# youmi-zym/GO-SLAM

Hardware: NVIDIA H100
Metric: keyframe-BA-updates/s (higher is better)
Workload: dtype f16 corr (f32 accumulate) / f32 BA (f64 solve)

## Files before the change

go-slam_b200/csrc/corr_build_tc.cu:

```cuda
#include "common.cuh"
#include "tc_ptx.cuh"
#include <mutex>
#include <cstdio>
#include <cuda.h>
#include <cstdlib>
#include <cstring>

int gs_corr_build_simt_f16(const __half* f1, const __half* f2, __half* const* levels,
                           int num_levels, int N, int D, int h, int w, cudaStream_t st);

namespace {

constexpr int kD = 128;
constexpr int kBM = 128;
constexpr int kPY = 8, kPX = 16;
constexpr int kKBox = 64;
constexpr int kTileBytes = kBM * kD * 2;
constexpr int kBoxBytes = kBM * kKBox * 2;
constexpr int kBStages = 2;
constexpr int kGroupWarps = 4;
constexpr int kEpiThreads = 2 * kGroupWarps * 32;
constexpr int kThreadsTC = kEpiThreads + 128;
constexpr int kProducerRegs = 40, kConsumerRegs = 232;
constexpr int kMaxXB = 8;
constexpr int kBarBytes = 1024;
constexpr int kL0HalfBytes = 64 * 2 * 128;
constexpr int kL1HalfBytes = 64 * 64;
constexpr int kXpRowWords = 68;
constexpr int kXpWarpBytes = 8 * kXpRowWords * 4;
constexpr int kFixedBytes = 1024 + kBarBytes + (1 + kBStages) * kTileBytes;
__host__ __device__ constexpr int pitch2_of(int n_xb) { return (n_xb * 16 + 31) / 32 * 32; }
__host__ __device__ constexpr int pool2_src_bytes(bool tiled, int n_xb) {
  return tiled ? pitch2_of(n_xb) + 48 : 2 * n_xb * 8 + 8;
}
__host__ __device__ constexpr int pool1_src_bytes(int n_xb) { return 4 * n_xb * 16 + 16; }
__host__ __device__ constexpr int smem_bytes(bool tiled, int n_xb) {
  return tiled ? kFixedBytes + 2 * kBStages * (kL0HalfBytes + kL1HalfBytes) + kBM * pool2_src_bytes(true, n_xb)
               : kFixedBytes + kBM * (pool1_src_bytes(n_xb) + pool2_src_bytes(false, n_xb)) +
                     kEpiThreads / 32 * kXpWarpBytes;
}
static_assert(smem_bytes(true, kMaxXB) <= 227 * 1024 && smem_bytes(false, kMaxXB) <= 227 * 1024,
              "corr_build_tc_kernel exceeds the 227 KB of shared memory of a block");

using namespace gs_tc;

struct TcParams {
  __half* lvl[4];
  int num_levels, N, h, w, hw;
  int n_mt, n_yb, n_xb;
  int n_items;
  const int64_t* ii; const int64_t* jj; int rig;
  const int* out_slot;
  int w4_0, h4_0, w4_1, h4_1;
  int pitch2, pitch3;
  int aligned;
  int experiment;
};

__device__ __forceinline__ uint32_t pack2(float a, float b) {
  const __half2 h = __floats2half2_rn(a, b);
  return *reinterpret_cast<const uint32_t*>(&h);
}
__device__ __forceinline__ float lo_f(uint32_t u) {
  return __half2float(__ushort_as_half((unsigned short)(u & 0xffffu)));
}
__device__ __forceinline__ float hi_f(uint32_t u) {
  return __half2float(__ushort_as_half((unsigned short)(u >> 16)));
}
__device__ __forceinline__ float pool_pair(uint32_t top, uint32_t bot) {
  float s = lo_f(top);
  s += hi_f(top);
  s += lo_f(bot);
  s += hi_f(bot);
  return s * 0.25f;
}
template <int NW>
__device__ __forceinline__ void store_row(__half* dst, const uint32_t (&r)[NW], int nvalid) {
  const uintptr_t a = reinterpret_cast<uintptr_t>(dst);
  if (nvalid >= 2 * NW) {
    if (NW == 8 && (a & 31) == 0) {
      asm volatile("st.global.v4.b32 [%0], {%1,%2,%3,%4}; st.global.v4.b32 [%0+16], {%5,%6,%7,%8};" ::"l"(dst), "r"(r[0]),
                   "r"(r[1]), "r"(r[2]), "r"(r[3]), "r"(r[4]), "r"(r[5]), "r"(r[6]), "r"(r[7])
                   : "memory");
      return;
    }
    if (NW >= 4 && (a & 15) == 0) {
#pragma unroll
      for (int i = 0; i < NW; i += 4)
        *reinterpret_cast<uint4*>(dst + 2 * i) = make_uint4(r[i], r[i + 1], r[i + 2], r[i + 3]);
      return;
    }
    if (NW == 2 && (a & 7) == 0) {
      *reinterpret_cast<uint2*>(dst) = make_uint2(r[0], r[1]);
      return;
    }
    if ((a & 3) == 0) {
#pragma unroll
      for (int i = 0; i < NW; ++i) *reinterpret_cast<uint32_t*>(dst + 2 * i) = r[i];
      return;
    }
  }
#pragma unroll
  for (int i = 0; i < NW; ++i) {
    if (2 * i < nvalid) dst[2 * i] = __ushort_as_half((unsigned short)(r[i] & 0xffffu));
    if (2 * i + 1 < nvalid) dst[2 * i + 1] = __ushort_as_half((unsigned short)(r[i] >> 16));
  }
}

__device__ __forceinline__ void tiled_half_epilogue(const float (&acc)[2][32], unsigned char* st0, unsigned char* st1,
                                                    unsigned char* pool2_row0, int p2src, int p2row, int xb,
                                                    int wrow, int lane) {
  uint32_t W[2][2][4][2];
#pragma unroll
  for (int rh = 0; rh < 2; ++rh)
#pragma unroll
    for (int ty = 0; ty < 2; ++ty)
#pragma unroll
      for (int r4 = 0; r4 < 4; ++r4)
#pragma unroll
        for (int jx = 0; jx < 2; ++jx) {
          const int j = 2 * r4 + jx;
          W[rh][ty][r4][jx] = pack2(acc[ty][4 * j + 2 * rh], acc[ty][4 * j + 2 * rh + 1]);
        }
  {
    const bool lo = (lane & 3) < 2;
    const bool dflip = (lane >> 4) & 1;
    const int s8 = lane & 7;
    const uint32_t st0_u = smem_u32(st0);
#pragma unroll
    for (int a = 0; a < 2; ++a)
#pragma unroll
      for (int k = 0; k < 2; ++k)
#pragma unroll
        for (int jx = 0; jx < 2; ++jx) {
          uint32_t m[4];
#pragma unroll
          for (int rh = 0; rh < 2; ++rh) {
            const uint32_t ra = dflip ? W[rh][a ^ 1][2 * k][jx] : W[rh][a][2 * k][jx];
            const uint32_t rb = dflip ? W[rh][a ^ 1][2 * k + 1][jx] : W[rh][a][2 * k + 1][jx];
            const uint32_t recv = __shfl_xor_sync(0xffffffffu, lo ? rb : ra, 2);
            m[2 * rh] = lo ? ra : recv;
            m[2 * rh + 1] = lo ? recv : rb;
          }
          const int tya = a ^ (s8 >> 2);
          const int R = 2 * (wrow + 8 * (lane >> 4) + s8) + tya;
          const int chunk = 2 * (2 * jx + ((lane >> 3) & 1)) + k;
          stmatrix_x4(st0_u + R * 128 + ((chunk ^ (R & 7)) << 4), m);
        }
  }
  const bool ev = (lane & 1) == 0;
  const uint32_t st1_u = smem_u32(st1);
#pragma unroll
  for (int rh = 0; rh < 2; ++rh) {
    const int s = wrow + 8 * rh + (lane >> 2);
#pragma unroll
    for (int jx = 0; jx < 2; ++jx) {
      float v[4];
#pragma unroll
      for (int ty = 0; ty < 2; ++ty)
#pragma unroll
        for (int k = 0; k < 2; ++k) v[2 * ty + k] = pool_pair(W[rh][ty][2 * k][jx], W[rh][ty][2 * k + 1][jx]);
      const uint32_t own01 = pack2(v[0], v[1]), own23 = pack2(v[2], v[3]);
      const uint32_t recv = __shfl_xor_sync(0xffffffffu, ev ? own23 : own01, 1);
      const uint32_t mine = ev ? own01 : own23;
      const uint32_t lo_w = ev ? mine : recv, hi_w = ev ? recv : mine;
      const uint32_t w0 = __byte_perm(lo_w, hi_w, 0x5410);
      const uint32_t w1 = __byte_perm(lo_w, hi_w, 0x7632);
      const int chunk = (2 * jx + (lane & 1)) ^ ((s >> 1) & 3);
      const uint32_t a1 = st1_u + s * 64 + (chunk << 4) + ((lane & 3) >> 1) * 4;
      st_shared_u32(a1 + (ev ? 0 : 8), ev ? w0 : w1);
      st_shared_u32(a1 + (ev ? 8 : 0), ev ? w1 : w0);
      const uint32_t l2 = pack2(pool_pair(w0, w1), 0.f);
      st_shared_u16(smem_u32(pool2_row0 + s * p2src + (lane & 1) * p2row + xb * 8 + (2 * jx + ((lane & 3) >> 1)) * 2),
                    (uint16_t)(l2 & 0xffffu));
    }
  }
}

template <bool kTiled>
__global__ void __launch_bounds__(kThreadsTC, 1)
corr_build_tc_kernel(const __grid_constant__ CUtensorMap mapA, const __grid_constant__ CUtensorMap mapB,
                     const __grid_constant__ CUtensorMap mapL0, const __grid_constant__ CUtensorMap mapL1,
                     const TcParams p) {
  extern __shared__ unsigned char smem_raw[];
  unsigned char* base = smem_raw + ((1024u - (smem_u32(smem_raw) & 1023u)) & 1023u);
  uint64_t* bars = reinterpret_cast<uint64_t*>(base);
  unsigned char* smA = base + kBarBytes;
  unsigned char* smB = smA + kTileBytes;
  unsigned char* smEpi = smB + kBStages * kTileBytes;
  uint64_t* full_a = bars;
  uint64_t* empty_a = bars + 1;
  uint64_t* full_b = bars + 2;
  uint64_t* empty_b = full_b + kBStages;

  const int warp = threadIdx.x >> 5, lane = threadIdx.x & 31;

  if (threadIdx.x == 0) {
    mbar_init(full_a, 1); mbar_init(empty_a, kEpiThreads / 32);
    for (int i = 0; i < kBStages; ++i) { mbar_init(&full_b[i], 1); mbar_init(&empty_b[i], kGroupWarps); }
    fence_barrier_init();
  }
  __syncthreads();

  if (warp >= kEpiThreads / 32) {
    setmaxnreg_dec<kProducerRegs>();
    if (warp == kEpiThreads / 32 && lane == 0) {
      int aph = 0, bs = 0, bph = 0;
      for (int item = blockIdx.x; item < p.n_items; item += gridDim.x) {
        const int yb = item % p.n_yb;
        const int mt = (item / p.n_yb) % p.n_mt;
        const int n = item / (p.n_yb * p.n_mt);
        int n1 = n, n2 = n;
        if (p.ii != nullptr) {
          const int fi = (int)p.ii[n], fj = (int)p.jj[n];
          n1 = p.rig * fi;
          n2 = p.rig * fj + ((fi == fj && p.rig > 1) ? 1 : 0);
        }
        mbar_wait(empty_a, aph ^ 1);
        mbar_expect_tx(full_a, kTileBytes);
        tma_load_3d(&mapA, full_a, smA, 0, mt * kBM, n1);
        tma_load_3d(&mapA, full_a, smA + kBoxBytes, kKBox, mt * kBM, n1);
        aph ^= 1;
        for (int xb = 0; xb < p.n_xb; ++xb) {
          mbar_wait(&empty_b[bs], bph ^ 1);
          mbar_expect_tx(&full_b[bs], kTileBytes);
          tma_load_4d(&mapB, &full_b[bs], smB + bs * kTileBytes, 0, xb * kPX, yb * kPY, n2);
          tma_load_4d(&mapB, &full_b[bs], smB + bs * kTileBytes + kBoxBytes, kKBox, xb * kPX,
                      yb * kPY, n2);
          if (++bs == kBStages) { bs = 0; bph ^= 1; }
        }
      }
    }
  } else {
    setmaxnreg_inc<kConsumerRegs>();
    const int group = warp >> 2;
    const int half = lane >> 4;
    const int etid = threadIdx.x;
    const int ts = group;
    unsigned char* smL0 = smEpi;
    unsigned char* smL1 = smL0 + 2 * kBStages * kL0HalfBytes;
    const int p1row = p.n_xb * 16, p1src = pool1_src_bytes(p.n_xb);
    const int p2row = p.n_xb * 8;
    const int p2src = pool2_src_bytes(kTiled, p.n_xb);
    unsigned char* pool1 = smEpi;
    unsigned char* pool2 = kTiled ? smL1 + 2 * kBStages * kL1HalfBytes : pool1 + kBM * p1src;
    unsigned char* smXp = pool2 + kBM * p2src;
    uint32_t* xp = reinterpret_cast<uint32_t*>(smXp + warp * kXpWarpBytes);
    const int h1 = p.h >> 1, w1 = p.w >> 1, h2 = p.h >> 2, w2 = p.w >> 2, h3 = p.h >> 3, w3 = p.w >> 3;
    const bool wr = p.experiment != 1;
    const bool tma_thread = (etid & 127) == 0;
    if (kTiled && etid < kBM) {
      for (int b = 2 * p2row; b < p.pitch2; b += 4)
        *reinterpret_cast<uint32_t*>(pool2 + etid * p2src + b) = 0u;
    }
    int aph = 0, bph = 0, tile = 0;
    for (int item = blockIdx.x; item < p.n_items; item += gridDim.x) {
      const int yb = item % p.n_yb;
      const int mt = (item / p.n_yb) % p.n_mt;
      const int n = item / (p.n_yb * p.n_mt);
      const int n_out = p.out_slot ? __ldg(p.out_slot + n) : n;
      const int y0 = yb * kPY;
      mbar_wait(full_a, aph);
      aph ^= 1;
      bool a_held = true;
      for (int xb = 0; xb < p.n_xb; ++xb, ++tile) {
        if ((tile & (kBStages - 1)) != ts) continue;
        const int x0 = xb * kPX;
        mbar_wait(&full_b[ts], bph);
        bph ^= 1;
        float acc[2][2][32];
        {
          const uint32_t a_addr = smem_u32(smA);
          const uint32_t b_addr = smem_u32(smB + ts * kTileBytes);
          wgmma_fence();
#pragma unroll
          for (int kb = 0; kb < kD / kKBox; ++kb) {
#pragma unroll
            for (int k = 0; k < kKBox / 16; ++k) {
              const uint64_t db = make_desc_sw128(b_addr + kb * kBoxBytes + k * 32);
              const uint32_t on = (kb | k) != 0 ? 1u : 0u;
#pragma unroll
              for (int mh = 0; mh < 2; ++mh) {
                const uint64_t da = make_desc_sw128(a_addr + mh * 64 * 128 + kb * kBoxBytes + k * 32);
                wgmma_m64n64(acc[mh][0], da, db, on);
                wgmma_m64n64(acc[mh][1], da, db + ((64 * 128) >> 4), on);
              }
            }
          }
          wgmma_commit();
          wgmma_wait<0>();
        }
        __syncwarp();
        if (lane == 0) {
          mbar_arrive(&empty_b[ts]);
          if (xb + kBStages >= p.n_xb) mbar_arrive(empty_a);
        }
        if (xb + kBStages >= p.n_xb) a_held = false;
#pragma unroll
        for (int mh = 0; mh < 2; ++mh) {
        if constexpr (kTiled) {
          unsigned char* st0 = smL0 + (group * 2 + mh) * kL0HalfBytes;
          unsigned char* st1 = smL1 + (group * 2 + mh) * kL1HalfBytes;
          tiled_half_epilogue(acc[mh], st0, st1, pool2 + mh * 64 * p2src, p2src, p2row, xb, (warp & 3) * 16, lane);
          fence_async_smem();
          if (tma_thread) bulk_wait_read<0>();
          named_bar_sync(1 + group, 128);
          if (tma_thread) {
            const int s0 = mt * kBM + mh * 64;
            if (wr && s0 < p.hw) {
              tma_store_4d(&mapL0, st0, xb * 64, 2 * yb, s0, n_out);
              if (p.num_levels > 1 && yb < p.h4_1) tma_store_4d(&mapL1, st1, xb * 32, yb, s0, n_out);
            }
            bulk_commit();
          }
        } else {
        const int row = mh * 64 + (warp & 3) * 16 + (lane & 15);
        const int src = mt * kBM + row;
        const bool src_ok = src < p.hw && wr;
        const long long plane_id = (long long)n_out * p.hw + src;
        uint32_t hr[4][8];
#pragma unroll
        for (int pass = 0; pass < 2; ++pass) {
#pragma unroll
          for (int sub = 0; sub < 2; ++sub)
#pragma unroll
            for (int j = 0; j < 8; ++j)
              xp[(lane >> 2) * kXpRowWords + sub * 32 + 4 * j + (lane & 3)] =
                  pack2(acc[mh][sub][4 * j + 2 * pass], acc[mh][sub][4 * j + 2 * pass + 1]);
          __syncwarp();
          if (((lane >> 3) & 1) == pass) {
            const uint4* sp = reinterpret_cast<const uint4*>(xp + (lane & 7) * kXpRowWords + half * 32);
#pragma unroll
            for (int i = 0; i < 8; ++i) {
              const uint4 v = sp[i];
              hr[i >> 1][4 * (i & 1)] = v.x; hr[i >> 1][4 * (i & 1) + 1] = v.y;
              hr[i >> 1][4 * (i & 1) + 2] = v.z; hr[i >> 1][4 * (i & 1) + 3] = v.w;
            }
          }
          __syncwarp();
        }
        uint32_t l1[2][4];
#pragma unroll
        for (int cc = 0; cc < 2; ++cc) {
          const int c = 2 * half + cc;
          if (src_ok) {
#pragma unroll
            for (int r = 0; r < 2; ++r) {
              const int y = y0 + 2 * c + r;
              if (y < p.h) store_row<8>(p.lvl[0] + (plane_id * p.h + y) * p.w + x0, hr[2 * cc + r], p.w - x0);
            }
          }
#pragma unroll
          for (int j = 0; j < 4; ++j)
            l1[cc][j] = pack2(pool_pair(hr[2 * cc][2 * j], hr[2 * cc + 1][2 * j]),
                              pool_pair(hr[2 * cc][2 * j + 1], hr[2 * cc + 1][2 * j + 1]));
          *reinterpret_cast<uint4*>(pool1 + row * p1src + c * p1row + xb * 16) =
              make_uint4(l1[cc][0], l1[cc][1], l1[cc][2], l1[cc][3]);
        }
        {
          const uint32_t a0 = pack2(pool_pair(l1[0][0], l1[1][0]), pool_pair(l1[0][1], l1[1][1]));
          const uint32_t a1 = pack2(pool_pair(l1[0][2], l1[1][2]), pool_pair(l1[0][3], l1[1][3]));
          *reinterpret_cast<uint2*>(pool2 + row * p2src + half * p2row + xb * 8) = make_uint2(a0, a1);
        }
        }
        }
      }
      if (a_held && lane == 0) mbar_arrive(empty_a);
      if (kTiled) fence_async_smem();
      named_bar_sync(3, kEpiThreads);
      if (wr && p.num_levels > 1)
      for (int s_loc = etid >> 2; s_loc < kBM; s_loc += kEpiThreads / 4) {
        const int part = etid & 3;
        const int s_glb = mt * kBM + s_loc;
        if (s_glb < p.hw) {
          const long long pl = (long long)n_out * p.hw + s_glb;
          const unsigned char* sp1 = pool1 + s_loc * p1src;
          const unsigned char* sp2 = pool2 + s_loc * p2src;
          if constexpr (kTiled) {
            if (part == 1 && p.num_levels > 2 && 2 * yb < h2) {
              bulk_store(reinterpret_cast<unsigned char*>(p.lvl[2]) + (pl * p.n_yb + yb) * (long long)p.pitch2, sp2,
                         (uint32_t)p.pitch2);
              bulk_commit();
              bulk_wait_read();
            }
            if (part == 2 && p.num_levels > 3 && yb < h3) {
              unsigned char* s3 = const_cast<unsigned char*>(sp2) + p.pitch2;
#pragma unroll
              for (int k = 0; k < 8; ++k) {
                uint32_t v = 0u;
                if (k < p.n_xb) {
                  const uint32_t t = *reinterpret_cast<const uint32_t*>(sp2 + 8 * k);
                  const uint32_t t2 = *reinterpret_cast<const uint32_t*>(sp2 + 8 * k + 4);
                  const uint32_t b = *reinterpret_cast<const uint32_t*>(sp2 + p2row + 8 * k);
                  const uint32_t b2 = *reinterpret_cast<const uint32_t*>(sp2 + p2row + 8 * k + 4);
                  v = pack2(pool_pair(t, b), pool_pair(t2, b2));
                }
                reinterpret_cast<uint32_t*>(s3)[k] = v;
              }
              fence_async_smem();
              bulk_store(reinterpret_cast<unsigned char*>(p.lvl[3]) + (pl * p.n_yb + yb) * 32LL, s3, 32u);
              bulk_commit();
              bulk_wait_read();
            }
          } else if (p.aligned) {
            unsigned char* g1 = reinterpret_cast<unsigned char*>(p.lvl[1]) +
                                (pl * h1 + (y0 >> 1)) * (long long)p1row;
            for (int off = part * 32; off < 4 * p1row; off += 128) {
              uint32_t rr[8];
#pragma unroll
              for (int k = 0; k < 8; ++k) rr[k] = *reinterpret_cast<const uint32_t*>(sp1 + off + 4 * k);
              asm volatile("st.global.v4.b32 [%0], {%1,%2,%3,%4}; st.global.v4.b32 [%0+16], {%5,%6,%7,%8};" ::"l"(g1 + off), "r"(rr[0]),
                           "r"(rr[1]), "r"(rr[2]), "r"(rr[3]), "r"(rr[4]), "r"(rr[5]), "r"(rr[6]), "r"(rr[7])
                           : "memory");
            }
            if (part == 1 && p.num_levels > 2) {
              unsigned char* g2 = reinterpret_cast<unsigned char*>(p.lvl[2]) +
                                  (pl * h2 + (y0 >> 2)) * (long long)p2row;
              for (int off = 0; off < 2 * p2row; off += 16)
                *reinterpret_cast<uint4*>(g2 + off) = make_uint4(
                    *reinterpret_cast<const uint32_t*>(sp2 + off), *reinterpret_cast<const uint32_t*>(sp2 + off + 4),
                    *reinterpret_cast<const uint32_t*>(sp2 + off + 8), *reinterpret_cast<const uint32_t*>(sp2 + off + 12));
            }
            if (part == 2 && p.num_levels > 3) {
              __half* g3 = p.lvl[3] + (pl * h3 + (y0 >> 3)) * w3;
              for (int x = 0; x < w3; x += 2) {
                const uint32_t t = *reinterpret_cast<const uint32_t*>(sp2 + 4 * x);
                const uint32_t t2 = *reinterpret_cast<const uint32_t*>(sp2 + 4 * x + 4);
                const uint32_t b = *reinterpret_cast<const uint32_t*>(sp2 + p2row + 4 * x);
                const uint32_t b2 = *reinterpret_cast<const uint32_t*>(sp2 + p2row + 4 * x + 4);
                *reinterpret_cast<uint32_t*>(g3 + x) = pack2(pool_pair(t, b), pool_pair(t2, b2));
              }
            }
          } else {
            const __half* s1 = reinterpret_cast<const __half*>(sp1);
            const __half* s2 = reinterpret_cast<const __half*>(sp2);
            for (int r = 0; r < 4; ++r) {
              const int y = (y0 >> 1) + r;
              if (y >= h1) break;
              __half* g = p.lvl[1] + (pl * h1 + y) * w1;
              for (int x = part; x < w1; x += 4) g[x] = s1[r * (p1row / 2) + x];
            }
            if (p.num_levels > 2)
              for (int r = 0; r < 2; ++r) {
                const int y = (y0 >> 2) + r;
                if (y >= h2) break;
                __half* g = p.lvl[2] + (pl * h2 + y) * w2;
                for (int x = part; x < w2; x += 4) g[x] = s2[r * (p2row / 2) + x];
              }
            if (p.num_levels > 3 && (y0 >> 3) < h3) {
              __half* g = p.lvl[3] + (pl * h3 + (y0 >> 3)) * w3;
              for (int x = part; x < w3; x += 4) {
                float sum = __half2float(s2[2 * x]);
                sum += __half2float(s2[2 * x + 1]);
                sum += __half2float(s2[(p2row / 2) + 2 * x]);
                sum += __half2float(s2[(p2row / 2) + 2 * x + 1]);
                g[x] = __float2half_rn(sum * 0.25f);
              }
// ... 11 lines not shown
to_kmajor_kernel(const __half* __restrict__ in, __half* __restrict__ out, int hw) {
  __shared__ __align__(16) __half tile[kD][64 + 2];
  const int n = blockIdx.y;
  const int p0 = blockIdx.x * 64;
  const __half* src = in + (size_t)n * kD * hw;
  const __half q = __float2half_rn(0.25f);
  if ((hw & 7) == 0 && p0 + 64 <= hw) {
    const __half2 q2 = __half2half2(q);
    for (int idx = threadIdx.x; idx < kD * 8; idx += 256) {
      const int k = idx >> 3, pp = (idx & 7) * 8;
      uint4 v = __ldg(reinterpret_cast<const uint4*>(src + (size_t)k * hw + p0 + pp));
      __half2* h = reinterpret_cast<__half2*>(&v);
      uint32_t* dstw = reinterpret_cast<uint32_t*>(&tile[k][pp]);
#pragma unroll
      for (int u = 0; u < 4; ++u) {
        const __half2 r = __hmul2(h[u], q2);
        dstw[u] = *reinterpret_cast<const uint32_t*>(&r);
      }
    }
  } else {
    for (int idx = threadIdx.x; idx < kD * 64; idx += 256) {
      const int k = idx / 64, pp = idx % 64;
      tile[k][pp] = (p0 + pp < hw) ? __hmul(src[(size_t)k * hw + p0 + pp], q) : __half(0.f);
    }
  }
  __syncthreads();
  __half* dst = out + ((size_t)n * hw + p0) * kD;
  for (int idx = threadIdx.x; idx < 64 * (kD / 2); idx += 256) {
    const int pp = idx / (kD / 2), k2 = idx % (kD / 2);
    if (p0 + pp < hw) {
      __half2 v = __halves2half2(tile[2 * k2][pp], tile[2 * k2 + 1][pp]);
      reinterpret_cast<__half2*>(dst + (size_t)pp * kD)[k2] = v;
    }
  }
}

typedef CUresult (*EncodeTiledFn)(CUtensorMap*, CUtensorMapDataType, cuuint32_t, void*,
                                  const cuuint64_t*, const cuuint64_t*, const cuuint32_t*,
                                  const cuuint32_t*, CUtensorMapInterleave, CUtensorMapSwizzle,
                                  CUtensorMapL2promotion, CUtensorMapFloatOOBfill);

EncodeTiledFn get_encode_fn() {
  static EncodeTiledFn fn = nullptr;
  if (fn) return fn;
  void* p = nullptr;
  cudaDriverEntryPointQueryResult q;
  if (cudaGetDriverEntryPoint("cuTensorMapEncodeTiled", &p, cudaEnableDefault, &q) != cudaSuccess ||
      q != cudaDriverEntryPointSuccess)
    return nullptr;
  fn = reinterpret_cast<EncodeTiledFn>(p);
  return fn;
}

#ifndef GOSLAM_TC_EXPERIMENT
#define GOSLAM_TC_EXPERIMENT 0
#endif
struct MapKey { const void* base; int F, h, w, kind; };
struct MapSlot { MapKey key; CUtensorMap map; unsigned long long stamp; bool used; };
constexpr int kMapSlots = 16;

bool encode_map(EncodeTiledFn enc, const MapKey& k, CUtensorMap* out) {
  const cuuint64_t hw = (cuuint64_t)k.h * k.w;
  if (k.kind == 0) {
    cuuint64_t dims[3] = {(cuuint64_t)kD, hw, (cuuint64_t)k.F};
    cuuint64_t strides[2] = {(cuuint64_t)kD * 2, hw * kD * 2};
    cuuint32_t box[3] = {(cuuint32_t)kKBox, (cuuint32_t)kBM, 1};
    cuuint32_t es[3] = {1, 1, 1};
    return enc(out, CU_TENSOR_MAP_DATA_TYPE_FLOAT16, 3, const_cast<void*>(k.base), dims, strides, box, es,
               CU_TENSOR_MAP_INTERLEAVE_NONE, CU_TENSOR_MAP_SWIZZLE_128B, CU_TENSOR_MAP_L2_PROMOTION_L2_128B,
               CU_TENSOR_MAP_FLOAT_OOB_FILL_NONE) == CUDA_SUCCESS;
  }
  if (k.kind >= 2) {
    const int lv = k.kind - 2;
    const cuuint64_t w4 = (cuuint64_t)gs_cdiv(k.w >> lv, 4), h4 = (cuuint64_t)gs_cdiv(k.h >> lv, 4);
    const cuuint64_t slot_bytes = hw * h4 * w4 * 32;
    cuuint64_t slots = ((cuuint64_t)1 << 40) / slot_bytes;
    if (slots > 0x7fffffffull) slots = 0x7fffffffull;
    cuuint64_t dims[4] = {w4 * 16, h4, hw, slots};
    cuuint64_t strides[3] = {w4 * 32, h4 * w4 * 32, slot_bytes};
    cuuint32_t box[4] = {lv == 0 ? 64u : 32u, lv == 0 ? 2u : 1u, 64u, 1u};
    cuuint32_t es[4] = {1, 1, 1, 1};
    return enc(out, CU_TENSOR_MAP_DATA_TYPE_FLOAT16, 4, const_cast<void*>(k.base), dims, strides, box, es,
               CU_TENSOR_MAP_INTERLEAVE_NONE, lv == 0 ? CU_TENSOR_MAP_SWIZZLE_128B : CU_TENSOR_MAP_SWIZZLE_64B,
               CU_TENSOR_MAP_L2_PROMOTION_NONE, CU_TENSOR_MAP_FLOAT_OOB_FILL_NONE) == CUDA_SUCCESS;
  }
  cuuint64_t dims[4] = {(cuuint64_t)kD, (cuuint64_t)k.w, (cuuint64_t)k.h, (cuuint64_t)k.F};
  cuuint64_t strides[3] = {(cuuint64_t)kD * 2, (cuuint64_t)k.w * kD * 2, hw * kD * 2};
  cuuint32_t box[4] = {(cuuint32_t)kKBox, (cuuint32_t)kPX, (cuuint32_t)kPY, 1};
  cuuint32_t es[4] = {1, 1, 1, 1};
  return enc(out, CU_TENSOR_MAP_DATA_TYPE_FLOAT16, 4, const_cast<void*>(k.base), dims, strides, box, es,
             CU_TENSOR_MAP_INTERLEAVE_NONE, CU_TENSOR_MAP_SWIZZLE_128B, CU_TENSOR_MAP_L2_PROMOTION_L2_128B,
             CU_TENSOR_MAP_FLOAT_OOB_FILL_NONE) == CUDA_SUCCESS;
}

bool cached_map(EncodeTiledFn enc, const MapKey& k, CUtensorMap* out) {
  static MapSlot table[kMapSlots];
  static unsigned long long clock = 0;
  static std::mutex mu;
  std::lock_guard<std::mutex> lock(mu);
  int victim = -1;
  for (int i = 0; i < kMapSlots; ++i) {
    MapSlot& s = table[i];
    if (s.used && s.key.base == k.base && s.key.F == k.F && s.key.h == k.h && s.key.w == k.w &&
        s.key.kind == k.kind) {
      s.stamp = ++clock;
      *out = s.map;
      return true;
    }
    if (victim < 0 || (table[victim].used && (!s.used || s.stamp < table[victim].stamp))) victim = i;
  }
  MapSlot& v = table[victim];
  if (!encode_map(enc, k, &v.map)) { v.used = false; return false; }
  v.key = k; v.used = true; v.stamp = ++clock;
  *out = v.map;
  return true;
}

int launch_tc(const __half* f1t, int F1, const __half* f2t, int F2, const int64_t* ii,
              const int64_t* jj, int rig, const int* out_slot, int tiled, __half* const* levels,
              int num_levels, int N, int h, int w, cudaStream_t st) {
  const int hw = h * w;
  EncodeTiledFn enc = get_encode_fn();
  if (!enc) return GOSLAM_ELAUNCH;
  CUtensorMap mapA, mapB, mapL0, mapL1;
  if (!cached_map(enc, MapKey{f1t, F1, h, w, 0}, &mapA) || !cached_map(enc, MapKey{f2t, F2, h, w, 1}, &mapB))
    return GOSLAM_ELAUNCH;
  mapL0 = mapL1 = mapA;
  if (tiled) {
    if ((reinterpret_cast<uintptr_t>(levels[0]) & 15) ||
        (num_levels > 1 && (reinterpret_cast<uintptr_t>(levels[1]) & 15)))
      return GOSLAM_EINVAL;
    if (!cached_map(enc, MapKey{levels[0], 0, h, w, 2}, &mapL0) ||
        (num_levels > 1 && !cached_map(enc, MapKey{levels[1], 0, h, w, 3}, &mapL1)))
      return GOSLAM_ELAUNCH;
  }
  TcParams p{};
  for (int i = 0; i < 4; ++i) p.lvl[i] = i < num_levels ? levels[i] : nullptr;
  p.num_levels = num_levels; p.N = N; p.h = h; p.w = w; p.hw = hw;
  p.n_mt = gs_cdiv(hw, kBM); p.n_yb = gs_cdiv(h, kPY); p.n_xb = gs_cdiv(w, kPX);
  p.n_items = N * p.n_mt * p.n_yb;
  p.ii = ii; p.jj = jj; p.rig = rig; p.out_slot = out_slot;
  p.w4_0 = gs_cdiv(w, 4); p.h4_0 = gs_cdiv(h, 4);
  p.w4_1 = gs_cdiv(w >> 1, 4); p.h4_1 = gs_cdiv(h >> 1, 4);
  p.pitch2 = pitch2_of(p.n_xb); p.pitch3 = 32;
  p.aligned = (w % 16 == 0 && h % 8 == 0) ? 1 : 0;
  p.experiment = GOSLAM_TC_EXPERIMENT;
  static int sm_count[64];
  static std::mutex dev_mu;
  int dev = 0;
  cudaGetDevice(&dev);
  if (dev < 0 || dev >= 64) dev = 0;
  int sms;
  {
    std::lock_guard<std::mutex> lock(dev_mu);
    if (sm_count[dev] == 0) {
      if (cudaFuncSetAttribute(corr_build_tc_kernel<true>, cudaFuncAttributeMaxDynamicSharedMemorySize,
                               smem_bytes(true, kMaxXB)) != cudaSuccess ||
          cudaFuncSetAttribute(corr_build_tc_kernel<false>, cudaFuncAttributeMaxDynamicSharedMemorySize,
                               smem_bytes(false, kMaxXB)) != cudaSuccess)
        return GOSLAM_ELAUNCH;
      int n = kNumSms;
      cudaDeviceGetAttribute(&n, cudaDevAttrMultiProcessorCount, dev);
      sm_count[dev] = n > 0 ? n : kNumSms;
    }
    sms = sm_count[dev];
  }
  const int grid = p.n_items < sms ? p.n_items : sms;
  const int smem = smem_bytes(tiled != 0, p.n_xb);
  if (tiled)
    corr_build_tc_kernel<true><<<grid, kThreadsTC, smem, st>>>(mapA, mapB, mapL0, mapL1, p);
  else
    corr_build_tc_kernel<false><<<grid, kThreadsTC, smem, st>>>(mapA, mapB, mapL0, mapL1, p);
  GS_CHECK_LAUNCH();
  return GOSLAM_OK;
}

int build_tc(const __half* f1, const __half* f2, __half* const* levels, int num_levels, int N,
             int h, int w, void* workspace, size_t workspace_bytes, cudaStream_t st) {
  const int hw = h * w;
  const size_t per = (size_t)N * hw * kD * sizeof(__half);
  if (workspace == nullptr || workspace_bytes < 2 * gs_align(per)) return GOSLAM_EWORKSPACE;
  __half* f1t = reinterpret_cast<__half*>(workspace);
  __half* f2t = reinterpret_cast<__half*>(reinterpret_cast<char*>(workspace) + gs_align(per));
  dim3 tg(gs_cdiv(hw, 64), N);
  to_kmajor_kernel<<<tg, 256, 0, st>>>(f1, f1t, hw);
  to_kmajor_kernel<<<tg, 256, 0, st>>>(f2, f2t, hw);
  GS_CHECK_LAUNCH();
  return launch_tc(f1t, N, f2t, N, nullptr, nullptr, 1, nullptr, 0, levels, num_levels, N, h, w, st);
}

}

extern "C" {

size_t goslam_corr_build_workspace_bytes(int N, int D, int h, int w) {
  if (N <= 0 || D != kD) return 256;
  return 2 * gs_align((size_t)N * h * w * kD * sizeof(__half)) + 256;
}

int goslam_fmaps_to_kmajor(const void* fmaps, void* out, int F, int D, int h, int w, void* stream) {
  if (F < 0 || D != kD || h <= 0 || w <= 0) return GOSLAM_EINVAL;
  if (F == 0) return GOSLAM_OK;
  dim3 tg(gs_cdiv(h * w, 64), F);
  to_kmajor_kernel<<<tg, 256, 0, (cudaStream_t)stream>>>(reinterpret_cast<const __half*>(fmaps),
                                                         reinterpret_cast<__half*>(out), h * w);
  GS_CHECK_LAUNCH();
  return GOSLAM_OK;
}

int goslam_corr_build_indexed(const void* fmaps_kmajor, int F, int rig, const int64_t* ii,
                              const int64_t* jj, void* const* levels, int num_levels, int N, int D,
                              int h, int w, void* stream) {
  return goslam_corr_pool_build(fmaps_kmajor, F, rig, ii, jj, nullptr, GOSLAM_LAYOUT_ROWMAJOR, levels,
                                num_levels, N, D, h, w, stream);
}

size_t goslam_corr_level_plane_elems(int level, int layout, int h, int w) {
  if (level < 0 || level > 3 || h <= 0 || w <= 0) return 0;
  const int hl = h >> level, wl = w >> level;
  if (hl <= 0 || wl <= 0) return 0;
  if (layout == GOSLAM_LAYOUT_TILED) {
    if (level < 2) return (size_t)gs_cdiv(hl, 4) * gs_cdiv(wl, 4) * 16;
    const int n_yb = gs_cdiv(h, kPY), n_xb = gs_cdiv(w, kPX);
    return level == 2 ? (size_t)n_yb * ((n_xb * 8 + 15) / 16 * 16) : (size_t)n_yb * 16;
  }
// ... 38 lines not shown
```

go-slam_b200/csrc/tc_ptx.cuh:

```cuda
#pragma once
#include <cuda.h>
#include <stdint.h>

namespace gs_tc {

__device__ __forceinline__ uint32_t smem_u32(const void* p) {
  return (uint32_t)__cvta_generic_to_shared(p);
}
__device__ __forceinline__ void mbar_init(uint64_t* bar, uint32_t count) {
  asm volatile("mbarrier.init.shared::cta.b64 [%0], %1;" ::"r"(smem_u32(bar)), "r"(count));
}
__device__ __forceinline__ void mbar_expect_tx(uint64_t* bar, uint32_t bytes) {
  asm volatile("mbarrier.arrive.expect_tx.shared::cta.b64 _, [%0], %1;" ::"r"(smem_u32(bar)),
               "r"(bytes) : "memory");
}
__device__ __forceinline__ void mbar_arrive(uint64_t* bar) {
  asm volatile("mbarrier.arrive.shared::cta.b64 _, [%0];" ::"r"(smem_u32(bar)) : "memory");
}
__device__ __forceinline__ void mbar_wait(uint64_t* bar, uint32_t parity) {
  const uint32_t addr = smem_u32(bar);
  uint32_t ok;
  do {
    asm volatile(
        "{\n\t"
        ".reg .pred p;\n\t"
        "mbarrier.try_wait.parity.shared::cta.b64 p, [%1], %2;\n\t"
        "selp.u32 %0, 1, 0, p;\n\t"
        "}\n"
        : "=r"(ok) : "r"(addr), "r"(parity) : "memory");
  } while (!ok);
}
__device__ __forceinline__ void fence_barrier_init() {
  asm volatile("fence.mbarrier_init.release.cluster;" ::: "memory");
}
__device__ __forceinline__ void tma_load_3d(const CUtensorMap* map, uint64_t* bar, void* dst,
                                            int c0, int c1, int c2) {
  asm volatile(
      "cp.async.bulk.tensor.3d.shared::cluster.global.mbarrier::complete_tx::bytes"
      " [%0], [%1, {%3, %4, %5}], [%2];" ::"r"(smem_u32(dst)), "l"((uint64_t)map),
      "r"(smem_u32(bar)), "r"(c0), "r"(c1), "r"(c2) : "memory");
}
__device__ __forceinline__ void tma_load_4d(const CUtensorMap* map, uint64_t* bar, void* dst,
                                            int c0, int c1, int c2, int c3) {
  asm volatile(
      "cp.async.bulk.tensor.4d.shared::cluster.global.mbarrier::complete_tx::bytes"
      " [%0], [%1, {%3, %4, %5, %6}], [%2];" ::"r"(smem_u32(dst)), "l"((uint64_t)map),
      "r"(smem_u32(bar)), "r"(c0), "r"(c1), "r"(c2), "r"(c3) : "memory");
}
__device__ __forceinline__ void bulk_store(void* gdst, const void* ssrc, uint32_t bytes) {
  asm volatile("cp.async.bulk.global.shared::cta.bulk_group [%0], [%1], %2;" ::"l"(gdst),
               "r"(smem_u32(ssrc)), "r"(bytes) : "memory");
}
__device__ __forceinline__ void tma_store_4d(const CUtensorMap* map, const void* ssrc, int c0, int c1, int c2,
                                             int c3) {
  asm volatile("cp.async.bulk.tensor.4d.global.shared::cta.bulk_group [%0, {%2, %3, %4, %5}], [%1];" ::"l"(
                   (uint64_t)map), "r"(smem_u32(ssrc)), "r"(c0), "r"(c1), "r"(c2), "r"(c3) : "memory");
}
__device__ __forceinline__ void bulk_commit() { asm volatile("cp.async.bulk.commit_group;" ::: "memory"); }
template <int N = 0>
__device__ __forceinline__ void bulk_wait_read() { asm volatile("cp.async.bulk.wait_group.read %0;" ::"n"(N) : "memory"); }
__device__ __forceinline__ void bulk_wait_all() { asm volatile("cp.async.bulk.wait_group 0;" ::: "memory"); }
__device__ __forceinline__ void fence_async_smem() { asm volatile("fence.proxy.async.shared::cta;" ::: "memory"); }
__device__ __forceinline__ void stmatrix_x4(uint32_t saddr, const uint32_t (&r)[4]) {
  asm volatile("stmatrix.sync.aligned.m8n8.x4.shared.b16 [%0], {%1, %2, %3, %4};" ::"r"(saddr), "r"(r[0]),
               "r"(r[1]), "r"(r[2]), "r"(r[3]) : "memory");
}
__device__ __forceinline__ void st_shared_u32(uint32_t saddr, uint32_t v) {
  asm volatile("st.shared.b32 [%0], %1;" ::"r"(saddr), "r"(v) : "memory");
}
__device__ __forceinline__ void st_shared_u16(uint32_t saddr, uint16_t v) {
  asm volatile("st.shared.b16 [%0], %1;" ::"r"(saddr), "h"(v) : "memory");
}
__device__ __forceinline__ void named_bar_sync(int id, int count) {
  asm volatile("bar.sync %0, %1;" ::"r"(id), "r"(count) : "memory");
}

__device__ __forceinline__ uint64_t make_desc_sw128(uint32_t saddr) {
  uint64_t d = 0;
  d |= (uint64_t)((saddr >> 4) & 0x3FFF);
  d |= (uint64_t)1 << 16;
  d |= (uint64_t)(1024 >> 4) << 32;
  d |= (uint64_t)1 << 62;
  return d;
}
template <int N>
__device__ __forceinline__ void setmaxnreg_inc() { asm volatile("setmaxnreg.inc.sync.aligned.u32 %0;" ::"n"(N)); }
template <int N>
__device__ __forceinline__ void setmaxnreg_dec() { asm volatile("setmaxnreg.dec.sync.aligned.u32 %0;" ::"n"(N)); }
__device__ __forceinline__ void wgmma_fence() { asm volatile("wgmma.fence.sync.aligned;" ::: "memory"); }
__device__ __forceinline__ void wgmma_commit() { asm volatile("wgmma.commit_group.sync.aligned;" ::: "memory"); }
template <int N>
__device__ __forceinline__ void wgmma_wait() { asm volatile("wgmma.wait_group.sync.aligned %0;" ::"n"(N) : "memory"); }

__device__ __forceinline__ void wgmma_m64n64(float (&d)[32], uint64_t da, uint64_t db, uint32_t accumulate) {
  asm volatile(
      "{\n\t"
      ".reg .pred p;\n\t"
      "setp.ne.b32 p, %34, 0;\n\t"
      "wgmma.mma_async.sync.aligned.m64n64k16.f32.f16.f16 "
      "{%0,%1,%2,%3,%4,%5,%6,%7,%8,%9,%10,%11,%12,%13,%14,%15,"
      "%16,%17,%18,%19,%20,%21,%22,%23,%24,%25,%26,%27,%28,%29,%30,%31}, %32, %33, p, 1, 1, 0, 0;\n\t"
      "}\n"
      : "+f"(d[0]), "+f"(d[1]), "+f"(d[2]), "+f"(d[3]), "+f"(d[4]), "+f"(d[5]), "+f"(d[6]), "+f"(d[7]),
        "+f"(d[8]), "+f"(d[9]), "+f"(d[10]), "+f"(d[11]), "+f"(d[12]), "+f"(d[13]), "+f"(d[14]), "+f"(d[15]),
        "+f"(d[16]), "+f"(d[17]), "+f"(d[18]), "+f"(d[19]), "+f"(d[20]), "+f"(d[21]), "+f"(d[22]), "+f"(d[23]),
        "+f"(d[24]), "+f"(d[25]), "+f"(d[26]), "+f"(d[27]), "+f"(d[28]), "+f"(d[29]), "+f"(d[30]), "+f"(d[31])
      : "l"(da), "l"(db), "r"(accumulate));
}
__device__ __forceinline__ void wgmma_m64n16(float (&d)[8], uint64_t da, uint64_t db, uint32_t accumulate) {
  asm volatile(
      "{\n\t"
      ".reg .pred p;\n\t"
      "setp.ne.b32 p, %10, 0;\n\t"
      "wgmma.mma_async.sync.aligned.m64n16k16.f32.f16.f16 "
      "{%0,%1,%2,%3,%4,%5,%6,%7}, %8, %9, p, 1, 1, 0, 0;\n\t"
      "}\n"
      : "+f"(d[0]), "+f"(d[1]), "+f"(d[2]), "+f"(d[3]), "+f"(d[4]), "+f"(d[5]), "+f"(d[6]), "+f"(d[7])
      : "l"(da), "l"(db), "r"(accumulate));
}

}
```

Baseline: 1431.

## Offload level-2/3 pyramid stores to dedicated store warps with double-buffered bands

Producer-side spare warps become store warps. They compute the level-3 pooling and issue TMA tensor stores for levels 2 and 3 from a double-buffered band, synchronised with the consumers through staged/freed mbarriers. The consumer warps no longer take the full named barrier plus per-row bulk stores. They now issue per-warp TMA stores for levels 0 and 1 with a 16-row box and up to three outstanding groups, and the level-0 store is issued between the level-0 and level-1 epilogue phases. L2 cache hints are added: evict_last on input loads and evict_first on the streaming output stores. The experiment switch also becomes a compile-time constant. Shared memory use grows and the synchronisation becomes more complex, which adds risk of hazards on buffer reuse.

```diff
diff --git a/go-slam_b200/csrc/corr_build_tc.cu b/go-slam_b200/csrc/corr_build_tc.cu
--- a/go-slam_b200/csrc/corr_build_tc.cu
+++ b/go-slam_b200/csrc/corr_build_tc.cu
@@ -23,19 +23,23 @@
 constexpr int kThreadsTC = kEpiThreads + 128;
 constexpr int kProducerRegs = 40, kConsumerRegs = 232;
 constexpr int kMaxXB = 8;
+constexpr int kStoreWarps = 3;
 constexpr int kBarBytes = 1024;
 constexpr int kL0HalfBytes = 64 * 2 * 128;
 constexpr int kL1HalfBytes = 64 * 64;
+constexpr int kL0WarpBytes = kL0HalfBytes / kGroupWarps, kL1WarpBytes = kL1HalfBytes / kGroupWarps;
+constexpr int kL3BandBytes = kBM * 32;
 constexpr int kXpRowWords = 68;
 constexpr int kXpWarpBytes = 8 * kXpRowWords * 4;
 constexpr int kFixedBytes = 1024 + kBarBytes + (1 + kBStages) * kTileBytes;
 __host__ __device__ constexpr int pitch2_of(int n_xb) { return (n_xb * 16 + 31) / 32 * 32; }
 __host__ __device__ constexpr int pool2_src_bytes(bool tiled, int n_xb) {
-  return tiled ? pitch2_of(n_xb) + 48 : 2 * n_xb * 8 + 8;
-}
+  return tiled ? pitch2_of(n_xb) : 2 * n_xb * 8 + 8;
+}
+__host__ __device__ constexpr int band_bytes(int n_xb) { return kBM * pool2_src_bytes(true, n_xb) + kL3BandBytes; }
 __host__ __device__ constexpr int pool1_src_bytes(int n_xb) { return 4 * n_xb * 16 + 16; }
 __host__ __device__ constexpr int smem_bytes(bool tiled, int n_xb) {
-  return tiled ? kFixedBytes + 2 * kBStages * (kL0HalfBytes + kL1HalfBytes) + kBM * pool2_src_bytes(true, n_xb)
+  return tiled ? kFixedBytes + 2 * kBStages * (kL0HalfBytes + kL1HalfBytes) + 2 * band_bytes(n_xb)
                : kFixedBytes + kBM * (pool1_src_bytes(n_xb) + pool2_src_bytes(false, n_xb)) +
                      kEpiThreads / 32 * kXpWarpBytes;
 }
@@ -54,8 +58,12 @@
   int w4_0, h4_0, w4_1, h4_1;
   int pitch2, pitch3;
   int aligned;
-  int experiment;
 };
+
+#ifndef GOSLAM_TC_EXPERIMENT
+#define GOSLAM_TC_EXPERIMENT 0
+#endif
+constexpr int kExperiment = GOSLAM_TC_EXPERIMENT;
 
 __device__ __forceinline__ uint32_t pack2(float a, float b) {
   const __half2 h = __floats2half2_rn(a, b);
@@ -107,9 +115,10 @@
   }
 }
 
+template <typename F>
 __device__ __forceinline__ void tiled_half_epilogue(const float (&acc)[2][32], unsigned char* st0, unsigned char* st1,
                                                     unsigned char* pool2_row0, int p2src, int p2row, int xb,
-                                                    int wrow, int lane) {
+                                                    int wrow, int lane, F between_levels) {
   uint32_t W[2][2][4][2];
 #pragma unroll
   for (int rh = 0; rh < 2; ++rh)
@@ -148,6 +157,7 @@
           stmatrix_x4(st0_u + R * 128 + ((chunk ^ (R & 7)) << 4), m);
         }
   }
+  between_levels();
   const bool ev = (lane & 1) == 0;
   const uint32_t st1_u = smem_u32(st1);
 #pragma unroll
@@ -181,6 +191,7 @@
 __global__ void __launch_bounds__(kThreadsTC, 1)
 corr_build_tc_kernel(const __grid_constant__ CUtensorMap mapA, const __grid_constant__ CUtensorMap mapB,
                      const __grid_constant__ CUtensorMap mapL0, const __grid_constant__ CUtensorMap mapL1,
+                     const __grid_constant__ CUtensorMap mapL2, const __grid_constant__ CUtensorMap mapL3,
                      const TcParams p) {
   extern __shared__ unsigned char smem_raw[];
   unsigned char* base = smem_raw + ((1024u - (smem_u32(smem_raw) & 1023u)) & 1023u);
@@ -192,12 +203,18 @@
   uint64_t* empty_a = bars + 1;
   uint64_t* full_b = bars + 2;
   uint64_t* empty_b = full_b + kBStages;
+  uint64_t* staged = empty_b + kBStages;
+  uint64_t* freed = staged + 2;
+  unsigned char* smL0 = smEpi;
+  unsigned char* smL1 = smL0 + 2 * kBStages * kL0HalfBytes;
+  constexpr bool wr = kExperiment != 1;
 
   const int warp = threadIdx.x >> 5, lane = threadIdx.x & 31;
 
   if (threadIdx.x == 0) {
     mbar_init(full_a, 1); mbar_init(empty_a, kEpiThreads / 32);
     for (int i = 0; i < kBStages; ++i) { mbar_init(&full_b[i], 1); mbar_init(&empty_b[i], kGroupWarps); }
+    for (int i = 0; i < 2; ++i) { mbar_init(&staged[i], kEpiThreads / 32); mbar_init(&freed[i], 1); }
     fence_barrier_init();
   }
   __syncthreads();
@@ -205,6 +222,7 @@
   if (warp >= kEpiThreads / 32) {
     setmaxnreg_dec<kProducerRegs>();
     if (warp == kEpiThreads / 32 && lane == 0) {
+      const uint64_t keep = l2_evict_last();
       int aph = 0, bs = 0, bph = 0;
       for (int item = blockIdx.x; item < p.n_items; item += gridDim.x) {
         const int yb = item % p.n_yb;
@@ -217,19 +235,65 @@
           n2 = p.rig * fj + ((fi == fj && p.rig > 1) ? 1 : 0);
         }
         mbar_wait(empty_a, aph ^ 1);
-        mbar_expect_tx(full_a, kTileBytes);
-        tma_load_3d(&mapA, full_a, smA, 0, mt * kBM, n1);
-        tma_load_3d(&mapA, full_a, smA + kBoxBytes, kKBox, mt * kBM, n1);
+        if constexpr (kExperiment == 2) {
+          mbar_arrive(full_a);
+        } else {
+          mbar_expect_tx(full_a, kTileBytes);
+          tma_load_3d_hint(&mapA, full_a, smA, 0, mt * kBM, n1, keep);
+          tma_load_3d_hint(&mapA, full_a, smA + kBoxBytes, kKBox, mt * kBM, n1, keep);
+        }
         aph ^= 1;
         for (int xb = 0; xb < p.n_xb; ++xb) {
           mbar_wait(&empty_b[bs], bph ^ 1);
-          mbar_expect_tx(&full_b[bs], kTileBytes);
-          tma_load_4d(&mapB, &full_b[bs], smB + bs * kTileBytes, 0, xb * kPX, yb * kPY, n2);
-          tma_load_4d(&mapB, &full_b[bs], smB + bs * kTileBytes + kBoxBytes, kKBox, xb * kPX,
-                      yb * kPY, n2);
+          if constexpr (kExperiment == 2) {
+            mbar_arrive(&full_b[bs]);
+          } else {
+            mbar_expect_tx(&full_b[bs], kTileBytes);
+            tma_load_4d_hint(&mapB, &full_b[bs], smB + bs * kTileBytes, 0, xb * kPX, yb * kPY, n2, keep);
+            tma_load_4d_hint(&mapB, &full_b[bs], smB + bs * kTileBytes + kBoxBytes, kKBox, xb * kPX,
+                             yb * kPY, n2, keep);
+          }
           if (++bs == kBStages) { bs = 0; bph ^= 1; }
         }
       }
+    } else if (kTiled && warp > kEpiThreads / 32) {
+      const int sid = threadIdx.x - (kEpiThreads + 32);
+      const int p2src = p.pitch2, p2row = p.n_xb * 8;
+      unsigned char* pool2 = smL1 + 2 * kBStages * kL1HalfBytes;
+      const int h2 = p.h >> 2, h3 = p.h >> 3;
+      int it = 0;
+      for (int item = blockIdx.x; item < p.n_items; item += gridDim.x, ++it) {
+        const int yb = item % p.n_yb;
+        const int mt = (item / p.n_yb) % p.n_mt;
+        const int n = item / (p.n_yb * p.n_mt);
+        const bool out2 = wr && p.num_levels > 2 && 2 * yb < h2, out3 = wr && p.num_levels > 3 && yb < h3;
+        unsigned char* s2 = pool2 + (it & 1) * band_bytes(p.n_xb);
+        const uint32_t s2_u = smem_u32(s2), s3_u = s2_u + kBM * p2src;
+        mbar_wait(&staged[it & 1], (it >> 1) & 1);
+        if (out3) {
+          for (int i = sid; i < kBM * 8; i += kStoreWarps * 32) {
+            const int k = i & 7;
+            uint32_t v = 0u;
+            if (k < p.n_xb) {
+              const uint32_t a = s2_u + (i >> 3) * p2src + 8 * k;
+              v = pack2(pool_pair(ld_shared_u32(a), ld_shared_u32(a + p2row)),
+                        pool_pair(ld_shared_u32(a + 4), ld_shared_u32(a + p2row + 4)));
+            }
+            st_shared_u32(s3_u + 4 * i, v);
+          }
+          fence_async_smem();
+        }
+        named_bar_sync(4, kStoreWarps * 32);
+        if (sid == 0) {
+          const int n_out = p.out_slot ? __ldg(p.out_slot + n) : n;
+          if (out2) tma_store_4d_hint(&mapL2, s2, 0, yb, mt * kBM, n_out, l2_evict_first());
+          if (out3) tma_store_4d_hint(&mapL3, s2 + kBM * p2src, 0, yb, mt * kBM, n_out, l2_evict_first());
+          bulk_commit();
+          bulk_wait_read<0>();
+          mbar_arrive(&freed[it & 1]);
+        }
+      }
+      if (sid == 0) bulk_wait_all();
     }
   } else {
     setmaxnreg_inc<kConsumerRegs>();
@@ -237,8 +301,6 @@
     const int half = lane >> 4;
     const int etid = threadIdx.x;
     const int ts = group;
-    unsigned char* smL0 = smEpi;
-    unsigned char* smL1 = smL0 + 2 * kBStages * kL0HalfBytes;
     const int p1row = p.n_xb * 16, p1src = pool1_src_bytes(p.n_xb);
     const int p2row = p.n_xb * 8;
     const int p2src = pool2_src_bytes(kTiled, p.n_xb);
@@ -247,14 +309,13 @@
     unsigned char* smXp = pool2 + kBM * p2src;
     uint32_t* xp = reinterpret_cast<uint32_t*>(smXp + warp * kXpWarpBytes);
     const int h1 = p.h >> 1, w1 = p.w >> 1, h2 = p.h >> 2, w2 = p.w >> 2, h3 = p.h >> 3, w3 = p.w >> 3;
-    const bool wr = p.experiment != 1;
-    const bool tma_thread = (etid & 127) == 0;
-    if (kTiled && etid < kBM) {
-      for (int b = 2 * p2row; b < p.pitch2; b += 4)
-        *reinterpret_cast<uint32_t*>(pool2 + etid * p2src + b) = 0u;
-    }
-    int aph = 0, bph = 0, tile = 0;
-    for (int item = blockIdx.x; item < p.n_items; item += gridDim.x) {
+    if (kTiled && etid < 2 * kBM) {
+      unsigned char* piece = pool2 + (etid >> 7) * band_bytes(p.n_xb) + (etid & (kBM - 1)) * p2src;
+      for (int b = 2 * p2row; b < p2src; b += 4) st_shared_u32(smem_u32(piece + b), 0u);
+    }
+    const uint64_t stream = l2_evict_first();
+    int aph = 0, bph = 0, tile = 0, it = 0;
+    for (int item = blockIdx.x; item < p.n_items; item += gridDim.x, ++it) {
       const int yb = item % p.n_yb;
       const int mt = (item / p.n_yb) % p.n_mt;
       const int n = item / (p.n_yb * p.n_mt);
@@ -263,13 +324,25 @@
       mbar_wait(full_a, aph);
       aph ^= 1;
       bool a_held = true;
+      unsigned char* band = pool2;
+      if constexpr (kTiled) {
+        band += (it & 1) * band_bytes(p.n_xb);
+        mbar_wait(&freed[it & 1], ((it >> 1) & 1) ^ 1);
+      }
       for (int xb = 0; xb < p.n_xb; ++xb, ++tile) {
         if ((tile & (kBStages - 1)) != ts) continue;
         const int x0 = xb * kPX;
         mbar_wait(&full_b[ts], bph);
         bph ^= 1;
         float acc[2][2][32];
-        {
+        if constexpr (kExperiment == 2) {
+#pragma unroll
+          for (int i = 0; i < 128; ++i) {
+            uint32_t z;
+            asm volatile("mov.b32 %0, 0;" : "=r"(z));
+            acc[i >> 6][(i >> 5) & 1][i & 31] = __uint_as_float(z);
+          }
+        } else {
           const uint32_t a_addr = smem_u32(smA);
           const uint32_t b_addr = smem_u32(smB + ts * kTileBytes);
           wgmma_fence();
@@ -301,16 +374,26 @@
         if constexpr (kTiled) {
           unsigned char* st0 = smL0 + (group * 2 + mh) * kL0HalfBytes;
           unsigned char* st1 = smL1 + (group * 2 + mh) * kL1HalfBytes;
-          tiled_half_epilogue(acc[mh], st0, st1, pool2 + mh * 64 * p2src, p2src, p2row, xb, (warp & 3) * 16, lane);
+          const int wq = warp & 3;
+          const int s0 = mt * kBM + mh * 64 + wq * 16;
+          const bool out0 = wr && s0 < p.hw;
+          if (lane == 0) bulk_wait_read<3>();
+          __syncwarp();
+          tiled_half_epilogue(acc[mh], st0, st1, band + mh * 64 * p2src, p2src, p2row, xb, wq * 16, lane, [&] {
+            fence_async_smem();
+            __syncwarp();
+            if (lane == 0) {
+              if (out0) tma_store_4d_hint(&mapL0, st0 + wq * kL0WarpBytes, xb * 64, 2 * yb, s0, n_out, stream);
+              bulk_commit();
+              bulk_wait_read<3>();
+            }
+            __syncwarp();
+          });
           fence_async_smem();
-          if (tma_thread) bulk_wait_read<0>();
-          named_bar_sync(1 + group, 128);
-          if (tma_thread) {
-            const int s0 = mt * kBM + mh * 64;
-            if (wr && s0 < p.hw) {
-              tma_store_4d(&mapL0, st0, xb * 64, 2 * yb, s0, n_out);
-              if (p.num_levels > 1 && yb < p.h4_1) tma_store_4d(&mapL1, st1, xb * 32, yb, s0, n_out);
-            }
+          __syncwarp();
+          if (lane == 0) {
+            if (out0 && p.num_levels > 1 && yb < p.h4_1)
+              tma_store_4d_hint(&mapL1, st1 + wq * kL1WarpBytes, xb * 32, yb, s0, n_out, stream);
             bulk_commit();
           }
         } else {
@@ -366,7 +449,12 @@
         }
       }
       if (a_held && lane == 0) mbar_arrive(empty_a);
-      if (kTiled) fence_async_smem();
+      if constexpr (kTiled) {
+        fence_async_smem();
+        __syncwarp();
+        if (lane == 0) mbar_arrive(&staged[it & 1]);
+        continue;
+      }
       named_bar_sync(3, kEpiThreads);
       if (wr && p.num_levels > 1)
       for (int s_loc = etid >> 2; s_loc < kBM; s_loc += kEpiThreads / 4) {
@@ -376,33 +464,7 @@
           const long long pl = (long long)n_out * p.hw + s_glb;
           const unsigned char* sp1 = pool1 + s_loc * p1src;
           const unsigned char* sp2 = pool2 + s_loc * p2src;
-          if constexpr (kTiled) {
-            if (part == 1 && p.num_levels > 2 && 2 * yb < h2) {
-              bulk_store(reinterpret_cast<unsigned char*>(p.lvl[2]) + (pl * p.n_yb + yb) * (long long)p.pitch2, sp2,
-                         (uint32_t)p.pitch2);
-              bulk_commit();
-              bulk_wait_read();
-            }
-            if (part == 2 && p.num_levels > 3 && yb < h3) {
-              unsigned char* s3 = const_cast<unsigned char*>(sp2) + p.pitch2;
-#pragma unroll
-              for (int k = 0; k < 8; ++k) {
-                uint32_t v = 0u;
-                if (k < p.n_xb) {
-                  const uint32_t t = *reinterpret_cast<const uint32_t*>(sp2 + 8 * k);
-                  const uint32_t t2 = *reinterpret_cast<const uint32_t*>(sp2 + 8 * k + 4);
-                  const uint32_t b = *reinterpret_cast<const uint32_t*>(sp2 + p2row + 8 * k);
-                  const uint32_t b2 = *reinterpret_cast<const uint32_t*>(sp2 + p2row + 8 * k + 4);
-                  v = pack2(pool_pair(t, b), pool_pair(t2, b2));
-                }
-                reinterpret_cast<uint32_t*>(s3)[k] = v;
-              }
-              fence_async_smem();
-              bulk_store(reinterpret_cast<unsigned char*>(p.lvl[3]) + (pl * p.n_yb + yb) * 32LL, s3, 32u);
-              bulk_commit();
-              bulk_wait_read();
-            }
-          } else if (p.aligned) {
+          if (p.aligned) {
             unsigned char* g1 = reinterpret_cast<unsigned char*>(p.lvl[1]) +
                                 (pl * h1 + (y0 >> 1)) * (long long)p1row;
             for (int off = part * 32; off < 4 * p1row; off += 128) {
@@ -520,12 +582,9 @@
   return fn;
 }
 
-#ifndef GOSLAM_TC_EXPERIMENT
-#define GOSLAM_TC_EXPERIMENT 0
-#endif
 struct MapKey { const void* base; int F, h, w, kind; };
 struct MapSlot { MapKey key; CUtensorMap map; unsigned long long stamp; bool used; };
-constexpr int kMapSlots = 16;
+constexpr int kMapSlots = 32;
 
 bool encode_map(EncodeTiledFn enc, const MapKey& k, CUtensorMap* out) {
   const cuuint64_t hw = (cuuint64_t)k.h * k.w;
@@ -538,6 +597,20 @@
                CU_TENSOR_MAP_INTERLEAVE_NONE, CU_TENSOR_MAP_SWIZZLE_128B, CU_TENSOR_MAP_L2_PROMOTION_L2_128B,
                CU_TENSOR_MAP_FLOAT_OOB_FILL_NONE) == CUDA_SUCCESS;
   }
+  if (k.kind >= 4) {
+    const int n_yb = gs_cdiv(k.h, kPY);
+    const cuuint64_t piece = k.kind == 4 ? (cuuint64_t)pitch2_of(gs_cdiv(k.w, kPX)) : 32;
+    const cuuint64_t slot_bytes = hw * n_yb * piece;
+    cuuint64_t slots = ((cuuint64_t)1 << 40) / slot_bytes;
+    if (slots > 0x7fffffffull) slots = 0x7fffffffull;
+    cuuint64_t dims[4] = {piece / 2, (cuuint64_t)n_yb, hw, slots};
+    cuuint64_t strides[3] = {piece, n_yb * piece, slot_bytes};
+    cuuint32_t box[4] = {(cuuint32_t)(piece / 2), 1u, (cuuint32_t)kBM, 1u};
+    cuuint32_t es[4] = {1, 1, 1, 1};
+    return enc(out, CU_TENSOR_MAP_DATA_TYPE_FLOAT16, 4, const_cast<void*>(k.base), dims, strides, box, es,
+               CU_TENSOR_MAP_INTERLEAVE_NONE, CU_TENSOR_MAP_SWIZZLE_NONE, CU_TENSOR_MAP_L2_PROMOTION_NONE,
+               CU_TENSOR_MAP_FLOAT_OOB_FILL_NONE) == CUDA_SUCCESS;
+  }
   if (k.kind >= 2) {
     const int lv = k.kind - 2;
     const cuuint64_t w4 = (cuuint64_t)gs_cdiv(k.w >> lv, 4), h4 = (cuuint64_t)gs_cdiv(k.h >> lv, 4);
@@ -546,7 +619,7 @@
     if (slots > 0x7fffffffull) slots = 0x7fffffffull;
     cuuint64_t dims[4] = {w4 * 16, h4, hw, slots};
     cuuint64_t strides[3] = {w4 * 32, h4 * w4 * 32, slot_bytes};
-    cuuint32_t box[4] = {lv == 0 ? 64u : 32u, lv == 0 ? 2u : 1u, 64u, 1u};
+    cuuint32_t box[4] = {lv == 0 ? 64u : 32u, lv == 0 ? 2u : 1u, 16u, 1u};
     cuuint32_t es[4] = {1, 1, 1, 1};
     return enc(out, CU_TENSOR_MAP_DATA_TYPE_FLOAT16, 4, const_cast<void*>(k.base), dims, strides, box, es,
                CU_TENSOR_MAP_INTERLEAVE_NONE, lv == 0 ? CU_TENSOR_MAP_SWIZZLE_128B : CU_TENSOR_MAP_SWIZZLE_64B,
@@ -590,17 +663,16 @@
   const int hw = h * w;
   EncodeTiledFn enc = get_encode_fn();
   if (!enc) return GOSLAM_ELAUNCH;
-  CUtensorMap mapA, mapB, mapL0, mapL1;
+  CUtensorMap mapA, mapB, mapL0, mapL1, mapL2, mapL3;
   if (!cached_map(enc, MapKey{f1t, F1, h, w, 0}, &mapA) || !cached_map(enc, MapKey{f2t, F2, h, w, 1}, &mapB))
     return GOSLAM_ELAUNCH;
-  mapL0 = mapL1 = mapA;
+  mapL0 = mapL1 = mapL2 = mapL3 = mapA;
   if (tiled) {
-    if ((reinterpret_cast<uintptr_t>(levels[0]) & 15) ||
-        (num_levels > 1 && (reinterpret_cast<uintptr_t>(levels[1]) & 15)))
-      return GOSLAM_EINVAL;
-    if (!cached_map(enc, MapKey{levels[0], 0, h, w, 2}, &mapL0) ||
-        (num_levels > 1 && !cached_map(enc, MapKey{levels[1], 0, h, w, 3}, &mapL1)))
-      return GOSLAM_ELAUNCH;
+    for (int i = 0; i < num_levels; ++i)
+      if (reinterpret_cast<uintptr_t>(levels[i]) & 15) return GOSLAM_EINVAL;
+    CUtensorMap* maps[4] = {&mapL0, &mapL1, &mapL2, &mapL3};
+    for (int i = 0; i < num_levels; ++i)
+      if (!cached_map(enc, MapKey{levels[i], 0, h, w, 2 + i}, maps[i])) return GOSLAM_ELAUNCH;
   }
   TcParams p{};
   for (int i = 0; i < 4; ++i) p.lvl[i] = i < num_levels ? levels[i] : nullptr;
@@ -612,7 +684,6 @@
   p.w4_1 = gs_cdiv(w >> 1, 4); p.h4_1 = gs_cdiv(h >> 1, 4);
   p.pitch2 = pitch2_of(p.n_xb); p.pitch3 = 32;
   p.aligned = (w % 16 == 0 && h % 8 == 0) ? 1 : 0;
-  p.experiment = GOSLAM_TC_EXPERIMENT;
   static int sm_count[64];
   static std::mutex dev_mu;
   int dev = 0;
@@ -636,9 +707,9 @@
   const int grid = p.n_items < sms ? p.n_items : sms;
   const int smem = smem_bytes(tiled != 0, p.n_xb);
   if (tiled)
-    corr_build_tc_kernel<true><<<grid, kThreadsTC, smem, st>>>(mapA, mapB, mapL0, mapL1, p);
+    corr_build_tc_kernel<true><<<grid, kThreadsTC, smem, st>>>(mapA, mapB, mapL0, mapL1, mapL2, mapL3, p);
   else
-    corr_build_tc_kernel<false><<<grid, kThreadsTC, smem, st>>>(mapA, mapB, mapL0, mapL1, p);
+    corr_build_tc_kernel<false><<<grid, kThreadsTC, smem, st>>>(mapA, mapB, mapL0, mapL1, mapL2, mapL3, p);
   GS_CHECK_LAUNCH();
   return GOSLAM_OK;
 }
diff --git a/go-slam_b200/csrc/tc_ptx.cuh b/go-slam_b200/csrc/tc_ptx.cuh
--- a/go-slam_b200/csrc/tc_ptx.cuh
+++ b/go-slam_b200/csrc/tc_ptx.cuh
@@ -56,6 +56,35 @@
   asm volatile("cp.async.bulk.tensor.4d.global.shared::cta.bulk_group [%0, {%2, %3, %4, %5}], [%1];" ::"l"(
                    (uint64_t)map), "r"(smem_u32(ssrc)), "r"(c0), "r"(c1), "r"(c2), "r"(c3) : "memory");
 }
+__device__ __forceinline__ uint64_t l2_evict_first() {
+  uint64_t p;
+  asm volatile("createpolicy.fractional.L2::evict_first.b64 %0, 1.0;" : "=l"(p));
+  return p;
+}
+__device__ __forceinline__ uint64_t l2_evict_last() {
+  uint64_t p;
+  asm volatile("createpolicy.fractional.L2::evict_last.b64 %0, 1.0;" : "=l"(p));
+  return p;
+}
+__device__ __forceinline__ void tma_load_3d_hint(const CUtensorMap* map, uint64_t* bar, void* dst, int c0, int c1,
+                                                 int c2, uint64_t policy) {
+  asm volatile(
+      "cp.async.bulk.tensor.3d.shared::cluster.global.mbarrier::complete_tx::bytes.L2::cache_hint"
+      " [%0], [%1, {%3, %4, %5}], [%2], %6;" ::"r"(smem_u32(dst)), "l"((uint64_t)map),
+      "r"(smem_u32(bar)), "r"(c0), "r"(c1), "r"(c2), "l"(policy) : "memory");
+}
+__device__ __forceinline__ void tma_load_4d_hint(const CUtensorMap* map, uint64_t* bar, void* dst, int c0, int c1,
+                                                 int c2, int c3, uint64_t policy) {
+  asm volatile(
+      "cp.async.bulk.tensor.4d.shared::cluster.global.mbarrier::complete_tx::bytes.L2::cache_hint"
+      " [%0], [%1, {%3, %4, %5, %6}], [%2], %7;" ::"r"(smem_u32(dst)), "l"((uint64_t)map),
+      "r"(smem_u32(bar)), "r"(c0), "r"(c1), "r"(c2), "r"(c3), "l"(policy) : "memory");
+}
+__device__ __forceinline__ void tma_store_4d_hint(const CUtensorMap* map, const void* ssrc, int c0, int c1, int c2,
+                                                  int c3, uint64_t policy) {
+  asm volatile("cp.async.bulk.tensor.4d.global.shared::cta.bulk_group.L2::cache_hint [%0, {%2, %3, %4, %5}], [%1], %6;"
+               ::"l"((uint64_t)map), "r"(smem_u32(ssrc)), "r"(c0), "r"(c1), "r"(c2), "r"(c3), "l"(policy) : "memory");
+}
 __device__ __forceinline__ void bulk_commit() { asm volatile("cp.async.bulk.commit_group;" ::: "memory"); }
 template <int N = 0>
 __device__ __forceinline__ void bulk_wait_read() { asm volatile("cp.async.bulk.wait_group.read %0;" ::"n"(N) : "memory"); }
@@ -70,6 +99,11 @@
 }
 __device__ __forceinline__ void st_shared_u16(uint32_t saddr, uint16_t v) {
   asm volatile("st.shared.b16 [%0], %1;" ::"r"(saddr), "h"(v) : "memory");
+}
+__device__ __forceinline__ uint32_t ld_shared_u32(uint32_t saddr) {
+  uint32_t v;
+  asm volatile("ld.shared.b32 %0, [%1];" : "=r"(v) : "r"(saddr) : "memory");
+  return v;
 }
 __device__ __forceinline__ void named_bar_sync(int id, int count) {
   asm volatile("bar.sync %0, %1;" ::"r"(id), "r"(count) : "memory");
```

After: 1655, median of 6. 15.6% higher.
